# nulltea/hyper-greco

Hardware: AMD Instinct MI355X
Metric: GKR prove ms, n=32768 k=16 Goldilocks; achieved HBM GB/s vs roofline (lower is better)
Workload: dtype u64; 1 GPU; GKR prove (sk_encryption_circuit.rs:444-457) of the BFV sk-enc circuit, n=32768 k=16 Goldilocks/GoldilocksExt2, a new witness every step (4 seeded synthetic witnesses in rotation), node tables resident in HBM; witnesses=4, n=32768, k=16, field=goldilocks, parallelism=dp1: one independent proof per GPU, no data-path collective, proof_bytes=149488

## Files before the change

### hyper-greco_amd/csrc/kernels.hip

```cpp
#include <hip/hip_runtime.h>
#include <cstring>
#include <algorithm>
#include <stdexcept>
#include <string>
#include <type_traits>
#include "kernels.hpp"
#include "gl_wide.hpp"
#include "derive_math.hpp"

namespace hg {
namespace dev {

constexpr int TPB = 256;

template <int CTRL, int ROW_MASK>
__device__ __forceinline__ u64 dpp_u64(u64 v) {
    u32 lo = (u32)__builtin_amdgcn_update_dpp(0, (int)(u32)v, CTRL, ROW_MASK, 0xF, false);
    u32 hi = (u32)__builtin_amdgcn_update_dpp(0, (int)(u32)(v >> 32), CTRL, ROW_MASK, 0xF, false);
    return ((u64)hi << 32) | lo;
}
__device__ __forceinline__ u64 wave_sum_u64(u64 v) {
    v = gl_add(v, dpp_u64<0x111, 0xF>(v));
    v = gl_add(v, dpp_u64<0x112, 0xF>(v));
    v = gl_add(v, dpp_u64<0x114, 0xF>(v));
// ... 408 lines not shown
    if (threadIdx.x == 0) for (int w = 1; w < nw; w++) v = e2_add(v, sm[w]);
    return v;
}

constexpr int SM_SLOTS = 96;
extern __shared__ E2 dyn_lds[];
template <int N>
__device__ __forceinline__ void block_sum_multi(E2 (&v)[N], E2* sm ) {
    const int lane = threadIdx.x & 63, wave = threadIdx.x >> 6, nw = (blockDim.x + 63) >> 6;
#pragma unroll
    for (int k = 0; k < N; k++) v[k] = wave_sum(v[k]);
    __syncthreads();
    if (lane == 0) {
#pragma unroll
        for (int k = 0; k < N; k++) sm[wave * N + k] = v[k];
    }
    __syncthreads();
    if (threadIdx.x == 0)
        for (int w = 1; w < nw; w++) {
#pragma unroll
            for (int k = 0; k < N; k++) v[k] = e2_add(v[k], sm[w * N + k]);
        }
}

__device__ __forceinline__ void part_store(E2* p, E2 v) {
    __hip_atomic_store(&p->c0, v.c0, __ATOMIC_RELAXED, __HIP_MEMORY_SCOPE_AGENT);
    __hip_atomic_store(&p->c1, v.c1, __ATOMIC_RELAXED, __HIP_MEMORY_SCOPE_AGENT);
}
__device__ __forceinline__ E2 part_load(const E2* p) {
    return e2(__hip_atomic_load(&p->c0, __ATOMIC_RELAXED, __HIP_MEMORY_SCOPE_AGENT), __hip_atomic_load(&p->c1, __ATOMIC_RELAXED, __HIP_MEMORY_SCOPE_AGENT));
}
__device__ __forceinline__ unsigned* tickets_of(E2* partials) { return reinterpret_cast<unsigned*>(partials + PARTIALS_E2); }
struct NoPost { __device__ __forceinline__ void operator()(E2*) const {} };
template <typename Post = NoPost>
__device__ __forceinline__ void finish_partials(E2* p, int per, unsigned* ticket, E2* __restrict__ out, E2* sm ,
                                                int nblocks = -1, Post post = Post()) {
    __shared__ unsigned s_last;
    if (nblocks < 0) nblocks = (int)gridDim.x;
    if (threadIdx.x == 0) {
#if !defined(HG_STRICT_TICKETS) && defined(__HIP_DEVICE_COMPILE__) && !defined(__gfx950__) && !defined(__gfx942__)
#error "the vmcnt-ordered ticket below is only valid on gfx942 / gfx950 (stores tracked by vmcnt, sc1 stores written through); build other architectures with -DHG_STRICT_TICKETS"
#endif
#ifdef HG_STRICT_TICKETS
        unsigned t = __hip_atomic_fetch_add(ticket, 1u, __ATOMIC_ACQ_REL, __HIP_MEMORY_SCOPE_AGENT);
#else
        asm volatile("s_waitcnt vmcnt(0)" ::: "memory");
        unsigned t = __hip_atomic_fetch_add(ticket, 1u, __ATOMIC_RELAXED, __HIP_MEMORY_SCOPE_AGENT);
#endif
        s_last = (t == (unsigned)nblocks - 1) ? 1u : 0u;
    }
    __syncthreads();
    if (!s_last) return;
    __builtin_amdgcn_fence(__ATOMIC_ACQUIRE, "agent");
    constexpr int PER_MAX = 6;
    for (int v0 = 0; v0 < per; v0 += PER_MAX) {
        E2 a[PER_MAX];
#pragma unroll
        for (int v = 0; v < PER_MAX; v++) a[v] = e2_zero();
        for (int b = threadIdx.x; b < nblocks; b += blockDim.x) {
            E2 t[PER_MAX];
#pragma unroll
            for (int v = 0; v < PER_MAX; v++) if (v0 + v < per) t[v] = part_load(p + (size_t)b * per + v0 + v);
#pragma unroll
            for (int v = 0; v < PER_MAX; v++) if (v0 + v < per) a[v] = e2_add(a[v], t[v]);
        }
#pragma unroll
        for (int v = 0; v < PER_MAX; v++) if (v0 + v < per) a[v] = block_sum_n(a[v], sm);
        if (threadIdx.x == 0) {
            if constexpr (!std::is_same<Post, NoPost>::value) post(a);
#pragma unroll
            for (int v = 0; v < PER_MAX; v++) if (v0 + v < per) out[v0 + v] = a[v];
        }
    }
    if (threadIdx.x == 0) __hip_atomic_store(ticket, 0u, __ATOMIC_RELAXED, __HIP_MEMORY_SCOPE_AGENT);
}

__device__ __forceinline__ void st_io(const StJob& J, int rd, const void*& in, size_t& in_stride, E2*& out) {
    const size_t h = (size_t)1 << (J.nvars - 1 - rd);
    if (rd == 0) { in = J.in; in_stride = J.in_stride; }
    else { in = J.buf[(rd - 1) & 1]; in_stride = 2 * h; }
    out = rd == J.nvars - 1 ? J.final_out : J.buf[rd & 1];
}

__device__ __forceinline__ int find_item(const StItem* __restrict__ items, int nitems, int blk) {
    const int l = threadIdx.x & 63;
    const int b0 = l < nitems ? items[l].blk0 : 0x7fffffff;
    const unsigned long long m = __ballot(b0 <= blk);
    return __builtin_amdgcn_readfirstlane(__popcll(m) - 1);
}
__device__ __forceinline__ int find_item128(const StItem* __restrict__ items, int nitems, int blk) {
    const int l = threadIdx.x & 63;
    const int b0 = l < nitems ? items[l].blk0 : 0x7fffffff, b1 = l + 64 < nitems ? items[l + 64].blk0 : 0x7fffffff;
    const unsigned long long m0 = __ballot(b0 <= blk), m1 = __ballot(b1 <= blk);
    return __builtin_amdgcn_readfirstlane(__popcll(m0) + __popcll(m1) - 1);
}
template <int KIND, typename T, bool SLOT = false, int MODE = 0>
__global__ __launch_bounds__(256) void k_st_step(const StJob* __restrict__ jobs, const StItem* __restrict__ items, int nitems,
                                                 const E2* __restrict__ chal, E2* __restrict__ partials, E2* __restrict__ res) {
    constexpr int NV = KIND == SC_GRANDPROD ? 3 : 2;
    const int y = find_item(items, nitems, blockIdx.x);
    const StItem& I = items[y];
    const StJob& J = jobs[I.job];
    const int h_log2 = I.h_log2, jb_log2 = I.jb_log2;
    const int rd = J.nvars - 1 - h_log2;
    const size_t half = (size_t)1 << h_log2;
    const int nblocks = I.nblk, bx = (int)blockIdx.x - I.blk0;
    const void* in = I.in; const size_t in_stride = I.in_stride; E2* out = I.out;
    E2* sm = dyn_lds;
    E2* red = dyn_lds + SM_SLOTS;
    E2 acc[NV];
#pragma unroll
    for (int t = 0; t < NV; t++) acc[t] = e2_zero();
    if (rd == 0) sc_round_body<KIND, T, true, SLOT>(reinterpret_cast<const T*>(in), in_stride, out, half, J.ntab, half, chal[J.r_off + rd], J.pw, J.pwr, jb_log2, red, acc, bx, nblocks, J.p0_only != 0, J.next_level,
                                                    SLOT ? &J : nullptr);
    else sc_round_body<KIND, T, false, false, true, MODE>(reinterpret_cast<const T*>(in), in_stride, out, half, J.ntab, half, chal[J.r_off + rd], J.pw, J.pwr, jb_log2, red, acc, bx, nblocks, J.p0_only != 0, nullptr,
                                                          J.mirror ? &J : nullptr);
    if constexpr (MODE == 1) return;
    E2* part = partials + (size_t)y * SC_MAX_BLOCKS * NV;
    block_sum_multi<NV>(acc, sm);
    if (threadIdx.x == 0) {
#pragma unroll
        for (int t = 0; t < NV; t++) {
            if (nblocks == 1) res[J.sums_slot + (size_t)rd * NV + t] = acc[t];
            else part_store(part + (size_t)bx * NV + t, acc[t]);
        }
    }
    if (nblocks > 1) finish_partials(part, NV, tickets_of(partials) + y * 32, res + J.sums_slot + (size_t)rd * NV, sm, nblocks);
}
__device__ __forceinline__ u64 limb_word(const u64* __restrict__ input, const uint8_t* __restrict__ seg_lookup, int seg_shift, size_t rows,
                                         const u64* lookup_mask, size_t j) {
    return j < rows ? input[j] & lookup_mask[seg_lookup[j >> seg_shift]] : 0;
}
__device__ __forceinline__ u32 limb_of(u64 word, int c) { return (u32)(word >> (16 * c)) & 0xFFFF; }
template <typename S>
__device__ __forceinline__ ulonglong2 limb_pair(const S& H, size_t j2, int c) {
    if (j2 >= H.rows) return make_ulonglong2(0, 0);
    const ulonglong2 w = *reinterpret_cast<const ulonglong2*>(H.input + j2);
    const u64 m = H.lookup_mask[H.seg_lookup[j2 >> H.seg_shift]];
    return make_ulonglong2(limb_of(w.x & m, c), limb_of(w.y & m, c));
}
LimbSrc limb_src(const LassoDev& L, const u64* input) {
    LimbSrc S;
    memset(&S, 0, sizeof(S));
    S.input = input; S.seg_lookup = L.seg_lookup; S.seg_shift = L.seg_shift; S.rows = L.rows;
    memcpy(S.lookup_mask, L.lookup_mask, sizeof(S.lookup_mask));
    return S;
}
template <bool MIRROR, bool RECOMP, bool SLOT = false>
#ifndef HG_HASH_SLOT_WAVES
#define HG_HASH_SLOT_WAVES 3
#endif
__global__ __launch_bounds__(256) __attribute__((amdgpu_waves_per_eu(SLOT ? HG_HASH_SLOT_WAVES : 3, SLOT ? HG_HASH_SLOT_WAVES : 3))) void k_gp_first_hash(const StJob* __restrict__ job, const StItem* __restrict__ item,
                                                       const E2* __restrict__ chal, E2* __restrict__ partials, E2* __restrict__ res) {
    const StJob& J = *job;
    const StItem& I = *item;
    const GpHashSrc& H = *J.hash_src;
    const int h_log2 = I.h_log2;
    const size_t half = (size_t)1 << h_log2;
    const size_t hN = half << 1;
    const size_t ntiles = half >> 8;
    const int nblocks = I.nblk, bx = (int)blockIdx.x;
    E2* __restrict__ out = I.out;
    const E2 r = chal[J.r_off];
    const bool p0_only = J.p0_only != 0;
    [[maybe_unused]] constexpr bool mirror = MIRROR;
    const u64 gamma = H.gamma, gamma2 = H.gamma2, tau = H.tau;
    E2 acc[3] = {e2_zero(), e2_zero(), e2_zero()};
    for (size_t tile = bx; tile < ntiles; tile += nblocks) {
        const size_t j = (tile << 8) + threadIdx.x;
        const size_t jo = dpos(j, half);
        GpFirstAcc A = gp_first_acc_zero();
        E2 Sx = e2_zero(), Sy = e2_zero();
        u64 p0 = 0, p2 = 0, p3 = 0;
        int cur_chunk = -1;
        u64 c0 = 0, c1 = 0, c2 = 0, c3 = 0;
        u32 a01 = 0, a23 = 0;
        u32 uses_lo = 0, uses_hi = 0;
        if constexpr (RECOMP) {
            if (2 * j < H.rows) uses_lo = (u32)H.lookup_uses[H.seg_lookup[(2 * j) >> H.seg_shift]];
            if (hN + 2 * j < H.rows) uses_hi = (u32)H.lookup_uses[H.seg_lookup[(hN + 2 * j) >> H.seg_shift]];
        }
        [[maybe_unused]] const int sp = SLOT ? (int)((tile << 9) >> H.seg_shift) : 0;
        for (int m = 0; m < (SLOT ? H.nslots : H.nmem); m++) {
            [[maybe_unused]] int slot_v = m;
            int mi = m;
            if constexpr (SLOT) {
                mi = H.rep[(size_t)m * H.npairs + sp];
                if (mi == 255) {
                    store_e2_nt(out + (size_t)(2 * m) * half + jo, e2_zero());
                    store_e2_nt(out + (size_t)(2 * m + 1) * half + jo, e2_zero());
                    continue;
                }
            }
            const GpHashMem M = H.mems[mi];
            if (M.chunk != cur_chunk) {
                cur_chunk = M.chunk;
                const u64* __restrict__ ts = H.ts[cur_chunk];
                ulonglong2 dl, dh;
                if (H.limb_sh) { dl = limb_pair(H, 2 * j, cur_chunk); dh = limb_pair(H, hN + 2 * j, cur_chunk); }
                else {
                    const u64* __restrict__ dim = H.dim[cur_chunk];
                    dl = *reinterpret_cast<const ulonglong2*>(dim + 2 * j); dh = *reinterpret_cast<const ulonglong2*>(dim + hN + 2 * j);
                }
                const ulonglong2 tl = *reinterpret_cast<const ulonglong2*>(ts + 2 * j), th = *reinterpret_cast<const ulonglong2*>(ts + hN + 2 * j);
                c0 = gl_sub(gl_add(dl.x, gl_mul_small(gamma2, (u32)tl.x)), tau); c1 = gl_sub(gl_add(dl.y, gl_mul_small(gamma2, (u32)tl.y)), tau);
                c2 = gl_sub(gl_add(dh.x, gl_mul_small(gamma2, (u32)th.x)), tau); c3 = gl_sub(gl_add(dh.y, gl_mul_small(gamma2, (u32)th.y)), tau);
                if constexpr (RECOMP) { a01 = (u32)dl.x | ((u32)dl.y << 16); a23 = (u32)dh.x | ((u32)dh.y << 16); }
            }
            u32 e0, e1, e2v, e3;
            if constexpr (RECOMP) {
// ... 708 lines not shown
    const size_t len = (size_t)1 << J.len_log2;
    const size_t idx = (size_t)blockIdx.x * blockDim.x + threadIdx.x;
    if (idx >= ((size_t)J.nrows + J.has_s) << J.len_log2) return;
    const int b = (int)(idx >> J.len_log2);
    const size_t p = idx & (len - 1);
    if (b == J.nrows) { J.out[((size_t)(2 * J.nrows) << J.len_log2) + p] = J.in[((size_t)(2 * J.nslots) << J.len_log2) + p]; return; }
    const size_t t = p < len / 2 ? 2 * p : 2 * (p - len / 2) + 1;
    const int sp = (int)(t >> J.sh);
    const int v = J.slot_of[(size_t)b * J.npairs + sp];
    const E2 l = J.in[((size_t)(2 * v) << J.len_log2) + p], r = J.in[((size_t)(2 * v + 1) << J.len_log2) + p];
    J.out[((size_t)(2 * b) << J.len_log2) + p] = b == 0 ? l : e2_mul(J.ratio[(size_t)b * J.npairs + sp], l);
    J.out[((size_t)(2 * b + 1) << J.len_log2) + p] = r;
}
void gp_slot_regroup_jobs(hipStream_t st, const SlotRegroupJob* jobs, int njobs, size_t max_entries) {
    if (njobs) k_gp_slot_regroup_jobs<<<dim3((unsigned)((max_entries + 255) / 256), (unsigned)njobs), 256, 0, st>>>(jobs);
}
SlotRegroupJob gp_slot_regroup_job(const E2* in, E2* out, const uint8_t* slot_of, const E2* ratio, int nrows, int nslots, int npairs, int len_log2, bool has_s) {
    int np_log2 = 0;
    while ((1 << np_log2) < npairs) np_log2++;
    SlotRegroupJob J;
    J.in = in; J.out = out; J.slot_of = slot_of; J.ratio = ratio; J.nrows = nrows; J.nslots = nslots; J.npairs = npairs; J.len_log2 = len_log2; J.sh = len_log2 - np_log2; J.has_s = has_s ? 1 : 0;
    return J;
}
void gp_slot_regroup(hipStream_t st, const E2* in, E2* out, const uint8_t* slot_of, const E2* ratio, int nrows, int nslots, int npairs, int len_log2, bool has_s) {
    int np_log2 = 0;
    while ((1 << np_log2) < npairs) np_log2++;
    const size_t n = ((size_t)nrows + (has_s ? 1 : 0)) << len_log2;
    k_gp_slot_regroup<<<(unsigned)((n + 255) / 256), 256, 0, st>>>(in, out, slot_of, ratio, nrows, nslots, npairs, len_log2, len_log2 - np_log2, has_s ? 1 : 0);
}
int st_tail_whole_rounds(int ntab, int h0) { return ((size_t)(2 * ntab) << h0) * sizeof(E2) <= ST_TAIL_LDS_BYTES ? 1 : 2; }
size_t st_tail_table_bytes(int ntab, int h0, bool fold_first) {
    const size_t l0 = (size_t)ntab << h0;
    return (fold_first && h0 >= 1 && st_tail_whole_rounds(ntab, h0) == 1 ? 2 * l0 : l0 + (l0 >> 1)) * sizeof(E2);
}
void st_tail(hipStream_t st, int kind, const StJob* jobs, const StItem* items, int nitems, size_t table_bytes, const E2* chal, E2* res, bool fold_first) {
    const size_t lds = (SM_SLOTS + 3 * ST_TAIL_THREADS) * sizeof(E2) + table_bytes;
    static const hipError_t a1 = hipFuncSetAttribute((const void*)k_st_tail<SC_GRANDPROD>, hipFuncAttributeMaxDynamicSharedMemorySize, (int)((SM_SLOTS + 3 * ST_TAIL_THREADS) * sizeof(E2) + ST_TAIL_LDS_BYTES));
    static const hipError_t a2 = hipFuncSetAttribute((const void*)k_st_tail<SC_COLLATION>, hipFuncAttributeMaxDynamicSharedMemorySize, (int)((SM_SLOTS + 3 * ST_TAIL_THREADS) * sizeof(E2) + ST_TAIL_LDS_BYTES));
    static const hipError_t a3 = hipFuncSetAttribute((const void*)k_st_tail<SC_GRANDPROD, true>, hipFuncAttributeMaxDynamicSharedMemorySize, (int)((SM_SLOTS + 3 * ST_TAIL_THREADS) * sizeof(E2) + ST_TAIL_LDS_BYTES));
    (void)a1; (void)a2; (void)a3;
    if (kind == SC_GRANDPROD && fold_first) k_st_tail<SC_GRANDPROD, true><<<nitems, ST_TAIL_THREADS, lds, st>>>(jobs, items, chal, res);
    else if (kind == SC_GRANDPROD) k_st_tail<SC_GRANDPROD><<<nitems, ST_TAIL_THREADS, lds, st>>>(jobs, items, chal, res);
    else k_st_tail<SC_COLLATION><<<nitems, ST_TAIL_THREADS, lds, st>>>(jobs, items, chal, res);
}

int st_plan_blocks(StItem* items, int nitems, bool rounds2) {
    size_t total = 0;
    for (int q = 0; q < nitems; q++) total += (size_t)1 << items[q].h_log2;
    int blk = 0;
    for (int q = 0; q < nitems; q++) {
        StItem& I = items[q];
        int jb = 8;
        if (!rounds2 && I.nrounds != 2) while (jb > 2 && (total << (8 - jb)) < st_min_threads()) jb--;
        if (jb > I.h_log2) jb = I.h_log2;
        const size_t ntiles = ((size_t)1 << I.h_log2) >> jb;
        I.jb_log2 = jb;
        I.blk0 = blk;
        I.nblk = (int)std::min<size_t>(ntiles, (size_t)st_max_blocks());
        blk += I.nblk;
    }
    return blk;
}
void st_step(hipStream_t st, int kind, bool base, const StJob* jobs, const StItem* items, int nitems, int grid, const E2* chal,
             E2* partials, E2* res, bool slot, int mode) {
    const int nv = kind == SC_GRANDPROD ? 3 : 2;
    const size_t lds = sc_lds_bytes(nv, 256);
    if (mode) {
        if (kind != SC_GRANDPROD || base || slot) throw std::runtime_error("st_step: split rounds are grand-product rounds on Ext2 tables");
        if (mode == 1) k_st_step<SC_GRANDPROD, E2, false, 1><<<grid, 256, lds, st>>>(jobs, items, nitems, chal, partials, res);
        else k_st_step<SC_GRANDPROD, E2, false, 2><<<grid, 256, lds, st>>>(jobs, items, nitems, chal, partials, res);
        return;
    }
    if (slot) {
        if (kind != SC_GRANDPROD || !base || nitems != 1) throw std::runtime_error("st_step: a slot-form first round is launched alone");
        k_st_step<SC_GRANDPROD, u64, true><<<grid, 256, lds, st>>>(jobs, items, nitems, chal, partials, res);
    } else if (kind == SC_GRANDPROD) {
        if (base) k_st_step<SC_GRANDPROD, u64><<<grid, 256, lds, st>>>(jobs, items, nitems, chal, partials, res);
        else k_st_step<SC_GRANDPROD, E2><<<grid, 256, lds, st>>>(jobs, items, nitems, chal, partials, res);
    } else {
        if (base) k_st_step<SC_COLLATION, u64><<<grid, 256, lds, st>>>(jobs, items, nitems, chal, partials, res);
        else k_st_step<SC_COLLATION, E2><<<grid, 256, lds, st>>>(jobs, items, nitems, chal, partials, res);
    }
}
void st_step2(hipStream_t st, int kind, const StJob* jobs, const StItem* items, int nitems, int grid, const E2* chal, E2* partials, E2* res) {
    if (kind == SC_GRANDPROD) k_st_step2<false><<<grid, 256, sc_lds_bytes(0, 256), st>>>(jobs, items, nitems, chal, partials, res);
    else k_col_step2<<<grid, 256, sc_lds_bytes(0, 256), st>>>(jobs, items, nitems, chal, partials, res);
}
static_assert(HG_TEST_ST_MAX_BLOCKS <= ST_SUMS_PART_BLOCKS && (size_t)ST_SUMS_MAX_ITEMS * ST_SUMS_PART_BLOCKS * 6 <= PARTIALS_E2 && ST_SUMS_MAX_ITEMS * 16 <= PARTIALS_TICKETS,
              "st_sums: the items of a launch share one partials buffer");
void st_sums(hipStream_t st, const StJob* jobs, const StItem* items, int nitems, int grid, const E2* chal, E2* partials, E2* res) {
    if (nitems > ST_SUMS_MAX_ITEMS) throw std::runtime_error("st_sums: too many items in one launch");
    k_st_step2<true><<<grid, 256, sc_lds_bytes(3, 256), st>>>(jobs, items, nitems, chal, partials, res);
}
__device__ __forceinline__ void ps_io(const PsJob& J, int rd, int rounds, int in_buf, int out_buf, int i, const void*& a, const E2*& b, E2*& oa, E2*& ob) {
    const size_t N = (size_t)1 << J.nvars;
    if (in_buf < 0) { a = J.a[i]; b = J.b[i]; }
    else { size_t len = N >> rd; a = J.bufa[in_buf] + (size_t)i * len; b = J.bufb[in_buf] + (size_t)i * len; }
    if (out_buf < 0) { oa = J.fin_a[i]; ob = J.fin_b[i]; }
    else { size_t len = N >> (rd + rounds); oa = J.bufa[out_buf] + (size_t)i * len; ob = J.bufb[out_buf] + (size_t)i * len; }
}

template <typename TA>
__device__ __forceinline__ void ps_round_body(const PsJob& J, int rd, int in_buf, int out_buf, size_t half, E2 r, int jb_log2, E2& a0, E2& a2,
                                              size_t first_tile, size_t tile_step) {
    using V = Val<TA>;
    const int BD = blockDim.x, tid = threadIdx.x;
    const int G = BD >> jb_log2;
    const int jj = tid & ((1 << jb_log2) - 1), g = tid >> jb_log2;
    const size_t ntiles = half >> jb_log2;
    WE2 w0 = we2_zero(), w2 = we2_zero();
    const FoldR fr = fold_r(r);
    bool touched = false;
    for (size_t tile = first_tile; tile < ntiles; tile += tile_step) {
        const size_t j = (tile << jb_log2) + jj;
        const size_t jo = dpos(j, half);
        for (int i = g; i < J.npairs; i += G) {
            touched = true;
            const void* pa; const E2* pb; E2* oa; E2* ob;
            ps_io(J, rd, 1, in_buf, out_buf, i, pa, pb, oa, ob);
            TA xa, ya;
            E2 xb, yb;
            if (in_buf < 0) {
                load_pair<TA>(reinterpret_cast<const TA*>(pa) + 2 * j, xa, ya);
                load_pair<E2>(pb + 2 * j, xb, yb);
            } else {
                load_xy<TA, false>(reinterpret_cast<const TA*>(pa), j, half, xa, ya);
                load_xy<E2, false>(pb, j, half, xb, yb);
            }
            TA da = V::sub(ya, xa);
            E2 db = e2_sub(yb, xb);
            E2 vb = e2_add(yb, db);
            TA va = V::add(ya, da);
            if constexpr (std::is_same<TA, u64>::value) {
                wmac2(w0.A, xb.c0, xa, w0.C, xb.c1, xa);
                wmac2(w2.A, vb.c0, va, w2.C, vb.c1, va);
                const WAcc f0 = wacc_mul_init(xa, fr.r0, da), f1 = wacc_mul_init(0, fr.r1, da);
                store_e2(oa + jo, e2(wreduce(f0), wreduce(f1)));
            } else {
                we2_mac(w0, xb, xa);
                we2_mac(w2, vb, va);
                store_e2(oa + jo, e2_fold_wide(xa, da, fr));
            }
            store_e2(ob + jo, e2_fold_wide(xb, db, fr));
        }
    }
    if (touched) {
        a0 = e2_add(a0, we2_reduce(w0));
        a2 = e2_add(a2, we2_reduce(w2));
    }
}

__device__ __forceinline__ int find_ps_item(const PsItem* __restrict__ items, int nitems, int blk) {
    const int l = threadIdx.x & 63;
    const int b0 = l < nitems ? items[l].blk0 : 0x7fffffff;
    const unsigned long long m = __ballot(b0 <= blk);
    return __builtin_amdgcn_readfirstlane(__popcll(m) - 1);
}
__global__ __launch_bounds__(256) void k_ps_one(const PsJob* __restrict__ jobs, const PsItem* __restrict__ items, int nitems,
                                                const E2* __restrict__ chal, E2* __restrict__ partials, E2* __restrict__ res) {
    const int y = find_ps_item(items, nitems, blockIdx.x);
    const PsItem& I = items[y];
    const PsJob& J = jobs[I.job];
    const int rd = I.rd;
    const int nblocks = I.nblk, bx = (int)blockIdx.x - I.blk0;
    E2* sm = dyn_lds;
    const size_t half = (size_t)1 << (J.nvars - 1 - rd);
// ... 2033 lines not shown
```

### hyper-greco_amd/csrc/kernels.hpp

```cpp
#pragma once
#include <hip/hip_runtime.h>
#include <algorithm>
#include "gl_field.hpp"

namespace hg {
namespace dev {

constexpr int SC_MAX_BLOCKS = 1024;
constexpr size_t PARTIALS_E2 = (size_t)SC_MAX_BLOCKS * 6 * 64;
constexpr int PARTIALS_TICKETS = 64 * 32;
constexpr size_t PARTIALS_BYTES = PARTIALS_E2 * sizeof(E2) + PARTIALS_TICKETS * sizeof(unsigned);
constexpr int PS_MAX_PAIRS = 32;
constexpr int PW_MAX = 128;
constexpr int PW_ENTRY_MAX = 64;

struct Powers { E2 v[PW_MAX]; };
constexpr int MAX_CLAIMS = 32;
struct ClaimSet {
    int n;
    int unit_alpha;
    size_t alpha_off;
    size_t point_off[MAX_CLAIMS];
};

enum ScKind { SC_COLLATION = 0, SC_GRANDPROD = 1 };

struct GpHashMem {
    const u64* ep;
    int chunk;
    int rd_row, wr_row;
    u32 cutoff;
    int mem;
};
struct GpHashSrc {
    const u64* dim[4];
    const u64* ts[4];
    const GpHashMem* mems;
    int nmem;
    u64 gamma, gamma2, tau;
    int seg_shift;
    size_t rows;
    const uint8_t* seg_lookup;
    u64 lookup_uses[32];
    const u64* input;
    int limb_sh;
    u64 lookup_mask[32];
    const uint8_t* slot_of;
    const uint8_t* rep;
    const E2* slotw;
    int npairs, nslots;
    const u64* emit_rd;
    const u64* emit_wr;
};
void gp_slot_regroup(hipStream_t st, const E2* in, E2* out, const uint8_t* slot_of, const E2* ratio, int nrows, int nslots, int npairs, int len_log2, bool has_s = true);
struct SlotRegroupJob { const E2* in; E2* out; const uint8_t* slot_of; const E2* ratio; int nrows, nslots, npairs, len_log2, sh, has_s; };
SlotRegroupJob gp_slot_regroup_job(const E2* in, E2* out, const uint8_t* slot_of, const E2* ratio, int nrows, int nslots, int npairs, int len_log2, bool has_s);
void gp_slot_regroup_jobs(hipStream_t st, const SlotRegroupJob* jobs, int njobs, size_t max_entries);
struct GpClaimEp {
    E2 mu;
    u64 c;
    int nb;
    int nread;
    int has_next, has_claims;
    size_t evals_slot, next_slot, claims_slot;
    const E2* winv;
    const E2* gnext;
};
struct StJob {
    const void* in;
    size_t in_stride;
    E2* buf[2];
    E2* final_out;
    const GpClaimEp* ep;
    int kind, ntab, nvars, base;
    int p0_only;
    const E2* slotw;
    const u64* emit_mask;
    int slot_ng, slot_shift;
    int mirror;
    E2 mk1, mk2;
    size_t r_off;
    size_t sums_slot;
    const GpHashSrc* hash_src;
    u64* next_level;
    E2 pw[PW_MAX];
    E2 pwr[PW_MAX];
};
struct StItem {
    int job;
    int h_log2;
    int jb_log2;
    int blk0, nblk;
    const void* in;
    size_t in_stride;
    E2* out;
    int rd, nrounds;
    int ntab;
};
int st_plan_blocks(StItem* items, int nitems, bool rounds2);
void st_step(hipStream_t st, int kind, bool base, const StJob* jobs, const StItem* items, int nitems, int grid, const E2* chal,
             E2* partials, E2* res, bool slot = false, int mode = 0);
void st_first_hash(hipStream_t st, const StJob* job, const StItem* item, int grid, bool mirror, bool recomp, const E2* chal, E2* partials, E2* res, bool slot = false);
void st_step2(hipStream_t st, int kind, const StJob* jobs, const StItem* items, int nitems, int grid, const E2* chal, E2* partials, E2* res);
constexpr int ST_SUMS_MAX_ITEMS = 128, ST_SUMS_PART_BLOCKS = 512;
void st_sums(hipStream_t st, const StJob* jobs, const StItem* items, int nitems, int grid, const E2* chal, E2* partials, E2* res);
int st_tail_h(int ntab, int nvars);
int st_tail_whole_rounds(int ntab, int h0);
size_t st_tail_table_bytes(int ntab, int h0, bool fold_first);
void st_tail(hipStream_t st, int kind, const StJob* jobs, const StItem* items, int nitems, size_t table_bytes, const E2* chal, E2* res, bool fold_first = false);
constexpr int ST_SUMS_PAIR_MAX_NB = 24;
constexpr int ST_STEP2_MIN_H = 9;

struct PsJob {
    const void* a[PS_MAX_PAIRS];
    const E2* b[PS_MAX_PAIRS];
    E2* fin_a[PS_MAX_PAIRS];
    E2* fin_b[PS_MAX_PAIRS];
    E2* bufa[2];
    E2* bufb[2];
    int npairs, nvars;
    int tail_rd;
    int tail_buf;
    size_t r_off;
    size_t sums_slot;
    int eq_n, eq_single;
    const E2* eq_scal;
    const E2* eq_lo;
    const E2* eq_suf;
    E2* bufA[2];
    E2* eqA0;
};
struct PsEqPoint {
    size_t point_off;
    int w, nvars;
    unsigned hib;
    int kmin;
    E2* lo;
    E2* suf;
};
inline int ps_eq_kmin(int nvars) { int k = nvars - 13 < 9 ? nvars - 13 : 9; return k < 0 ? 0 : k; }
inline size_t ps_eq_lo_entries(int nvars) { return nvars > 8 ? (size_t)(nvars - 8) * 384 : 0; }
inline size_t ps_eq_suf_entries(int nvars) { return ((size_t)2 << (nvars - ps_eq_kmin(nvars))) - 1; }
constexpr int PS_EQ_MAX_VARS = 26;
void ps_eq_prep(hipStream_t st, const PsEqPoint* pts, int npts, const E2* chal);
void ps_eq_A(hipStream_t st, const PsJob* jobs, const int* ids, int nids, size_t max_quads);
struct PsItem {
    int job, jb_log2, blk0, nblk;
    int rd;
    int in_buf, out_buf;
    int pad;
};
int ps_plan_blocks(PsItem* items, int nitems, const PsJob* host_jobs, bool rounds2);
void ps_round(hipStream_t st, bool rounds2, const PsJob* jobs, const PsItem* items, int nitems, int grid, const E2* chal, E2* partials, E2* res, bool eq = false);
void ps_tail(hipStream_t st, const PsJob* jobs, int njobs, const E2* chal, E2* res);
size_t ps_tail_items_max();

struct ScatterEnt { const E2* src; size_t dst; };
void scatter_e2(hipStream_t st, const ScatterEnt* ents, size_t n, E2* dst_base);
void set_e2(hipStream_t st, E2* dst, E2 v);
void stamp(hipStream_t st, unsigned long long* slot);
struct ClearSet { unsigned* p[4]; size_t n[4]; };
void clear_words(hipStream_t st, const ClearSet& c);

void reduce_partials(hipStream_t st, const E2* partials, int nblocks, int nv, E2* out);

struct EqJob {
    E2* out;
    int n;
    const E2* point_dev;
    ClaimSet cs;
    E2* ab;
    int blk0, rows;
    int pblk0;
};
void eq_jobs(hipStream_t st, const EqJob* jobs, int njobs, int max_n, const E2* chal);
__host__ __device__ inline size_t eq_ab_entries(int n) { return 256 + ((size_t)1 << (n > 8 ? n - 8 : 0)); }
struct EqAbGrid { int prep, fill; };
EqAbGrid eq_ab_plan(EqJob* host_jobs, int njobs);
void eq_jobs_ab(hipStream_t st, const EqJob* jobs, int njobs, EqAbGrid grid, const E2* chal);
void eq_jobs_prep(hipStream_t st, const EqJob* jobs, int njobs, EqAbGrid grid, const E2* chal);
void sum_tables(hipStream_t st, E2* out, const E2* tabs, int ntabs, size_t n);

struct LassoDev {
    int nu, alpha, num_lookups, seg_shift;
    size_t rows;
    const uint8_t* seg_lookup;
    u64 lookup_mask[32];
// ... 112 lines not shown
```

### hyper-greco_amd/csrc/prover_sumcheck.inc

```

    static constexpr size_t TAIL_ITEMS = 4096;

    bool hash_recomp = false;
    std::vector<dev::StJob> st_jobs;
    std::vector<int> st_seq;
    std::vector<SlotPlan> st_slot;
    std::vector<int> st_credit_ntab;
    std::vector<double> st_fused_bytes;
    std::vector<std::function<void()>> st_after_seq;
    double pending_level_design = 0, pending_hash_reads = -1, hash_design_reads = 0;
    std::vector<double> st_level_design, st_hash_reads;
    double pending_fused_bytes = 0;
    double pending_fused_model_extra = 0, hash_model_extra = 0;
    std::vector<double> st_fused_model_extra;
    std::vector<dev::ScatterEnt> scatter;
    struct GpEpReq { int job = -1; dev::GpClaimEp ep; std::vector<E2> winv, gnext; };
    std::vector<GpEpReq> gp_eps;

    ScHandle sc_stride(int kind, const void* in, bool base, size_t in_stride, int ntab, int nvars, const dev::Powers& pw, E2* final_out,
                       bool enqueue = true, bool p0_only = false, int seq = 0, u64* next_level = nullptr, const dev::GpHashSrc* hash_src = nullptr,
                       const MirrorSpec* mirror = nullptr, int model_ntab = 0, const SlotPlan* slots = nullptr) {
        ScHandle h;
        h.nv = kind == dev::SC_GRANDPROD ? 3 : 2;
        h.nvars = nvars;
// ... 99 lines not shown
                    it.job = q; it.h_log2 = next_h[q]; it.in = cur_in[q]; it.in_stride = cur_stride[q]; it.out = J.buf[0];
                    lall.items.push_back(it);
                    cur_in[q] = it.out; cur_stride[q] = (size_t)1 << next_h[q];
                    next_h[q]--;
                }
                if (!lall.items.empty()) plan.push_back(lall);
            }
            static const bool no_split = hg_env_on("HG_NO_SPLIT");
            constexpr int split_h = 14;
            const bool may_split = kind == dev::SC_GRANDPROD && !no_split && st == ctx->stream && fork_recorded && world == 1;
            Launch lsum{kind, false, -1, false, 1, {}};
            lsum.mode = 2;
            for (;;) {
                Launch le{kind, false, -1, false, 1, {}}, l2{kind, false, -1, false, 2, {}};
                bool le_small = may_split;
                for (int q = 0; q < nj; q++) {
                    const dev::StJob& J = st_jobs[q];
                    const int h = next_h[q];
                    if (J.kind != kind || h <= h_small[q]) continue;
                    const bool first = J.nvars - 1 == h;
                    if (first && J.hash_src) throw Error("hash-source job without a sequenced first round");
                    dev::StItem it;
                    memset(&it, 0, sizeof(it));
                    it.job = q; it.h_log2 = h; it.in = cur_in[q]; it.in_stride = cur_stride[q];
                    it.out = first ? J.buf[0] : next_out(q);
                    const bool pair = !first && h - 1 > h_small[q] && h >= std::max(dev::ST_STEP2_MIN_H, fuse_min_h);
                    (pair ? l2 : le).items.push_back(it);
                    if (!pair && (first || h > split_h)) le_small = false;
                    next_h[q] = h - (pair ? 2 : 1);
                    cur_in[q] = it.out; cur_stride[q] = (size_t)1 << (pair ? h - 1 : h);
                }
                if (le.items.empty() && l2.items.empty()) break;
                if (!l2.items.empty()) plan.push_back(l2);
                if (!le.items.empty()) {
                    if (le_small) {
                        le.mode = 1;
                        for (auto& it : le.items) {
                            E2* fresh = ctx->alloc_n<E2>((size_t)st_jobs[it.job].ntab << it.h_log2);
                            it.out = fresh;
                            cur_in[it.job] = fresh;
                            lsum.items.push_back(it);
                        }
                    }
                    plan.push_back(le);
                }
            }
            if (!lsum.items.empty()) {
                if (!hg_env_on("HG_SUMS_SINGLE")) {
                    std::vector<dev::StItem> byjob = lsum.items;
                    std::stable_sort(byjob.begin(), byjob.end(), [](const dev::StItem& a, const dev::StItem& b) { return a.job < b.job; });
                    for (size_t k = 0; k < byjob.size(); k++) {
                        dev::StItem it = byjob[k];
                        if (k + 1 < byjob.size() && byjob[k + 1].job == it.job && byjob[k + 1].h_log2 == it.h_log2 - 1 && it.h_log2 >= dev::ST_STEP2_MIN_H &&
                            st_jobs[it.job].ntab / 2 <= dev::ST_SUMS_PAIR_MAX_NB) { it.nrounds = 2; k++; n_sum_pairs++; }
                        else n_sum_singles++;
                        lsum.run.push_back(it);
                    }
                } else n_sum_singles += (int)lsum.items.size();
                plan.push_back(lsum);
            }
            {
                Launch lc{kind, false, 0, true, 0, {}};
                for (int q = 0; q < nj; q++) {
                    const dev::StJob& J = st_jobs[q];
                    if (J.kind != kind || next_h[q] < 0) continue;
                    const int hs = next_h[q];
                    dev::StItem it;
                    memset(&it, 0, sizeof(it));
                    it.job = q; it.in = cur_in[q]; it.in_stride = cur_stride[q];
                    it.rd = J.nvars - 1 - hs; it.nrounds = hs + 1; it.out = J.final_out;
                    if (st_slot[q].tail_ntab) {
                        const SlotPlan& sp = st_slot[q];
                        if (cur_stride[q] != (size_t)2 << hs) throw Error("slot-form job: unexpected table length at the tail");
                        E2* rg = ctx->alloc_n<E2>((size_t)sp.tail_ntab << (hs + 1));
                        regroups.push_back(Regroup{q, (const E2*)cur_in[q], rg, hs + 1});
                        it.in = rg; it.ntab = sp.tail_ntab;
                    }
                    lc.items.push_back(it);
                    next_h[q] = -1;
                }
                if (!lc.items.empty()) plan.push_back(lc);
            }
        }
        if (hg_debug("plan"))
            for (const Launch& L : plan) {
                if (L.after_seq) { fprintf(stderr, "[hg plan] stride kind=%d after_seq=1\n", L.kind); continue; }
                int lo = INT_MAX, hi = INT_MIN;
                for (const dev::StItem& it : L.items) { const int v = L.tail ? it.nrounds : it.h_log2; lo = std::min(lo, v); hi = std::max(hi, v); }
                fprintf(stderr, "[hg plan] stride kind=%d base=%d nrounds=%d mode=%d tail=%d hash=%d items=%zu %s=%d..%d\n", L.kind, L.base ? 1 : 0, L.nrounds,
                        L.mode, L.tail ? 1 : 0, L.hash ? 1 : 0, L.items.size(), L.tail ? "rounds" : "h", lo, hi);
            }
        if (!gp_eps.empty()) {
            std::vector<E2> wts;
            std::vector<dev::GpClaimEp> eps;
            for (const GpEpReq& e : gp_eps) {
                if (e.job < 0 || e.job >= nj || st_jobs[e.job].kind != dev::SC_GRANDPROD) throw Error("grand product: claim epilogue without its job");
                wts.insert(wts.end(), e.winv.begin(), e.winv.end());
                wts.insert(wts.end(), e.gnext.begin(), e.gnext.end());
            }
            E2* d_wts = ctx->alloc_n<E2>(wts.size());
            dev::GpClaimEp* d_eps = ctx->alloc_n<dev::GpClaimEp>(gp_eps.size());
            size_t o = 0;
            for (size_t i = 0; i < gp_eps.size(); i++) {
                dev::GpClaimEp ep = gp_eps[i].ep;
                ep.winv = d_wts + o; o += gp_eps[i].winv.size();
                ep.gnext = d_wts + o; o += gp_eps[i].gnext.size();
                eps.push_back(ep);
                st_jobs[gp_eps[i].job].ep = d_eps + i;
            }
            upload(d_wts, wts.data(), wts.size() * sizeof(E2), "upload claim weights");
            upload(d_eps, eps.data(), eps.size() * sizeof(dev::GpClaimEp), "upload claim epilogues");
            gp_eps.clear();
        }
        dev::StJob* d_jobs = ctx->alloc_n<dev::StJob>(nj);
        upload(d_jobs, st_jobs.data(), (size_t)nj * sizeof(dev::StJob), "upload jobs");
        std::vector<dev::StItem> flat;
        std::vector<size_t> offs;
        std::vector<std::vector<int>> grids(plan.size());
        for (size_t li = 0; li < plan.size(); li++) {
            Launch& L = plan[li];
            std::vector<dev::StItem>& its = L.run.empty() ? L.items : L.run;
            const size_t batch = L.run.empty() ? MAX_BATCH : (size_t)dev::ST_SUMS_MAX_ITEMS;
            if (!L.tail && !L.after_seq)
                for (size_t o = 0; o < its.size(); o += batch)
                    grids[li].push_back(dev::st_plan_blocks(its.data() + o, (int)std::min<size_t>(batch, its.size() - o), L.nrounds == 2));
            offs.push_back(flat.size());
            flat.insert(flat.end(), its.begin(), its.end());
        }
        dev::StItem* d_items = ctx->alloc_n<dev::StItem>(flat.size());
        upload(d_items, flat.data(), flat.size() * sizeof(dev::StItem), "upload step items");
        auto round_bytes = [&](int q, int rd, bool model) {
            const dev::StJob& J = st_jobs[q];
            size_t half = (size_t)1 << (J.nvars - 1 - rd);
            return (double)(model ? st_credit_ntab[q] : J.ntab) * (2.0 * half * ((J.base && rd == 0) ? 8 : 16) + half * 16.0);
        };
        auto design_bytes = [&](int q, int rd, int nrounds, bool tail) {
            const dev::StJob& J = st_jobs[q];
            const size_t half = (size_t)1 << (J.nvars - 1 - rd);
            double b = (double)J.ntab * 2.0 * half * ((J.base && rd == 0) ? 8 : 16);
            if (rd == 0 && st_hash_reads[q] >= 0) b = st_hash_reads[q];
            if (!tail) b += (double)J.ntab * (double)(half >> (nrounds - 1)) * 16.0;
            if (rd == 0) b += st_level_design[q];
            return b;
        };
        for (size_t li = 0; li < plan.size(); li++) {
            const Launch& L = plan[li];
            if (L.kind == dev::SC_GRANDPROD && st_before_gp) { stamp("collation done"); st_before_gp(); st_before_gp = nullptr; stamp("grand products may start"); }
            if (L.after_seq) {
                for (auto& f : st_after_seq) f();
                st_after_seq.clear();
                if (st_before_gp2) { st_before_gp2(); st_before_gp2 = nullptr; }
                continue;
            }
            const std::vector<dev::StItem>& its = L.run.empty() ? L.items : L.run;
            const size_t batch = L.run.empty() ? MAX_BATCH : (size_t)dev::ST_SUMS_MAX_ITEMS;
            for (size_t o = 0; o < its.size(); o += batch) {
                const int cnt = (int)std::min<size_t>(batch, its.size() - o);
                double bytes = 0, model = 0;
                if (L.hash) {
                    const dev::StItem& it = its[o];
                    bytes = round_bytes(it.job, 0, false) + st_fused_bytes[it.job];
                    model = round_bytes(it.job, 0, true) + st_fused_bytes[it.job] + st_fused_model_extra[it.job];
                    ctx->prof_begin(cls_gp_hash, bytes, model, design_bytes(it.job, 0, 1, false));
                    dev::st_first_hash(st, d_jobs + it.job, d_items + offs[li] + o, grids[li][0], st_jobs[it.job].mirror != 0, hash_recomp, ctx->d_chal, partials, d_res(), st_slot[it.job].tail_ntab != 0);
                    ctx->prof_end();
                    stamp("first hash round done");
                    continue;
                }
                if (L.tail) {
                    size_t table_bytes = 0;
                    double design = 0;
                    const bool tail_ff = L.kind == dev::SC_GRANDPROD && !hg_env_on("HG_TAIL_WHOLE_ROUNDS");
                    std::vector<dev::SlotRegroupJob> rg_jobs;
                    size_t rg_max = 0;
                    for (int q = 0; q < cnt; q++) {
                        const dev::StItem& it = its[o + q];
                        const dev::StJob& J = st_jobs[it.job];
                        for (int k = 0; k < it.nrounds; k++) { bytes += round_bytes(it.job, it.rd + k, false); model += round_bytes(it.job, it.rd + k, true); }
                        design += (double)(it.ntab > 0 ? it.ntab : J.ntab) * 2.0 * (double)((size_t)1 << (J.nvars - 1 - it.rd)) * ((J.base && it.rd == 0) ? 8 : 16);
                        const int h0 = J.nvars - 1 - it.rd, tn = it.ntab > 0 ? it.ntab : J.ntab;
                        table_bytes = std::max(table_bytes, dev::st_tail_table_bytes(tn, h0, tail_ff));
                        if (tail_ff && it.nrounds > dev::st_tail_whole_rounds(tn, h0)) n_tail_ff++;
                        else if (L.kind == dev::SC_GRANDPROD) n_tail_whole++;
                        for (const Regroup& g : regroups) if (g.job == it.job) {
                            const SlotPlan& sp = st_slot[it.job];
                            rg_jobs.push_back(dev::gp_slot_regroup_job(g.in, g.out, sp.d_slot_of, sp.d_ratio, sp.nrows, sp.nslots, sp.npairs, g.len_log2, (sp.tail_ntab & 1) != 0));
                            rg_max = std::max(rg_max, ((size_t)sp.nrows + (sp.tail_ntab & 1)) << g.len_log2);
                        }
                    }
                    if (!rg_jobs.empty()) {
                        dev::SlotRegroupJob* d_rg = ctx->alloc_n<dev::SlotRegroupJob>(rg_jobs.size());
                        upload(d_rg, rg_jobs.data(), rg_jobs.size() * sizeof(dev::SlotRegroupJob), "upload regroup jobs");
                        dev::gp_slot_regroup_jobs(st, d_rg, (int)rg_jobs.size(), rg_max);
                    }
                    ctx->prof_begin(cls_tail, bytes, model, design);
                    dev::st_tail(st, L.kind, d_jobs, d_items + offs[li] + o, cnt, table_bytes, ctx->d_chal, d_res(), tail_ff);
                    ctx->prof_end();
                } else {
                    double design = 0;
                    for (int q = 0; q < cnt; q++) {
                        const dev::StItem& it = its[o + q];
                        const dev::StJob& J = st_jobs[it.job];
                        design += design_bytes(it.job, J.nvars - 1 - it.h_log2, L.nrounds, false);
                        for (int k = 0; k < L.nrounds; k++) { bytes += round_bytes(it.job, J.nvars - 1 - it.h_log2 + k, false); model += round_bytes(it.job, J.nvars - 1 - it.h_log2 + k, true); }
                        if (L.base && it.h_log2 == J.nvars - 1) { bytes += st_fused_bytes[it.job]; model += st_fused_bytes[it.job]; }
                    }
                    const int grid = grids[li][o / batch];
                    int cls = L.kind == dev::SC_GRANDPROD ? (L.base ? cls_gp_base : (L.nrounds == 2 ? cls_gp_ext2 : cls_gp_ext)) : (L.base ? cls_col_base : (L.nrounds == 2 ? cls_col_ext2 : cls_col_ext));
                    if (L.mode == 2) {
                        if (o == 0) {
                            hip_check(hipEventRecord(ctx->ev_sum[0], st), "split rounds: folds done");
                            hip_check(hipStreamWaitEvent(ctx->stream_sum, ctx->ev_sum[0], 0), "split rounds: wait for the folds");
                        }
                        ctx->prof_stream = ctx->stream_sum;
                        ctx->prof_begin(cls_gp_sums, 0, 0, design);
                        if (!L.run.empty()) dev::st_sums(ctx->stream_sum, d_jobs, d_items + offs[li] + o, cnt, grid, ctx->d_chal, ctx->d_partials4, d_res());
                        else dev::st_step(ctx->stream_sum, L.kind, false, d_jobs, d_items + offs[li] + o, cnt, grid, ctx->d_chal, ctx->d_partials4, d_res(), false, 2);
                        ctx->prof_end();
                        ctx->prof_stream = st;
                        if (o + batch >= its.size()) {
                            hip_check(hipEventRecord(ctx->ev_sum[1], ctx->stream_sum), "split rounds: sums done");
                            ctx->sum_pending = true;
                        }
                        continue;
                    }
                    ctx->prof_begin(cls, bytes, model, design);
                    if (L.nrounds == 2) dev::st_step2(st, L.kind, d_jobs, d_items + offs[li] + o, cnt, grid, ctx->d_chal, partials, d_res());
                    else dev::st_step(st, L.kind, L.base, d_jobs, d_items + offs[li] + o, cnt, grid, ctx->d_chal, partials, d_res(),
                                      L.base && st_jobs[its[o].job].slotw != nullptr, L.mode);
                    ctx->prof_end();
                }
            }
        }
        if (hg_debug("endgame") && (n_tail_ff || n_tail_whole || n_sum_pairs || n_sum_singles))
            fprintf(stderr, "[hg endgame] stride tail_fold_first=%d tail_whole=%d sums_pairs=%d sums_singles=%d\n", n_tail_ff, n_tail_whole, n_sum_pairs, n_sum_singles);
        if (st_before_gp) { st_before_gp(); st_before_gp = nullptr; }
        if (st_before_gp2) { st_before_gp2(); st_before_gp2 = nullptr; }
        st_jobs.clear();
        st_seq.clear();
        st_credit_ntab.clear();
        st_slot.clear();
        st_fused_bytes.clear();
        st_fused_model_extra.clear();
        st_level_design.clear();
        st_hash_reads.clear();
        for (auto& f : st_after_seq) f();
        st_after_seq.clear();
        if (!scatter.empty()) {
            dev::ScatterEnt* d = ctx->alloc_n<dev::ScatterEnt>(scatter.size());
            upload(d, scatter.data(), scatter.size() * sizeof(dev::ScatterEnt), "upload scatter list");
            dev::scatter_e2(st, d, scatter.size(), d_res());
            scatter.clear();
        }
    }

    std::map<int, std::vector<dev::PsJob>> ps_queue;
    std::vector<std::function<void()>> second_wave;

    ScHandle sc_prodsum(const std::vector<const u64*>& a, const std::vector<const E2*>& b, int nvars,
                        const std::vector<E2*>& fin_a, const std::vector<E2*>& fin_b, bool enqueue = true) {
        ScHandle h;
        h.nv = 2;
        h.nvars = nvars;
        h.point_off = epos();
        h.sums_slot = slot((size_t)nvars * 2);
        if (!enqueue) {
            for (int i = 0; i < nvars; i++) h.rs.push_back(squeeze());
            return h;
        }
        const int np = (int)a.size();
        if (np > dev::PS_MAX_PAIRS) throw Error("prodsum: too many table pairs");
        const size_t N = (size_t)1 << nvars;
        dev::PsJob J;
        memset(&J, 0, sizeof(J));
        J.npairs = np; J.nvars = nvars; J.r_off = h.point_off; J.sums_slot = h.sums_slot;
        for (int q = 0; q < 2; q++) {
            J.bufa[q] = ctx->alloc_n<E2>((size_t)np * std::max<size_t>(N >> (q + 1), 1));
            J.bufb[q] = ctx->alloc_n<E2>((size_t)np * std::max<size_t>(N >> (q + 1), 1));
        }
        for (int i = 0; i < np; i++) { J.a[i] = a[i]; J.b[i] = b[i]; J.fin_a[i] = fin_a[i]; J.fin_b[i] = fin_b[i]; }
        for (int i = 0; i < nvars; i++) h.rs.push_back(squeeze());
        ps_queue[nvars].push_back(J);
        return h;
    }
    static bool ps_eq_on() { static const bool v = !hg_env_on("HG_NO_PS_EQ"); return v; }
    static size_t ps_tail_items() { return std::min<size_t>(TAIL_ITEMS, dev::ps_tail_items_max()); }
    static int eq_tail_rd(int npairs, int nvars) {
        if (npairs < 1 || npairs > dev::PS_MAX_PAIRS || nvars > dev::PS_EQ_MAX_VARS) return -1;
        const size_t N = (size_t)1 << nvars;
        int rd = 0;
        while (rd < nvars && ((N >> rd) / 2) * (size_t)npairs > ps_tail_items()) rd++;
        if (rd & 1) rd++;
        if (rd < 2 || rd > nvars - 8 || rd < dev::ps_eq_kmin(nvars)) return -1;
        return rd;
    }
    std::vector<E2> eq_scal_host;
    std::vector<dev::PsEqPoint> eqpt_queue;
    std::map<std::tuple<size_t, int, int, unsigned>, std::pair<E2*, E2*>> eqpt_shared;
    ScHandle sc_prodsum_eq(const std::vector<const u64*>& a, const std::vector<E2>& kappa, const std::vector<E2>& zp, size_t z_off, int w, unsigned hib,
                           int nvars, int tail_rd, const std::vector<E2*>& fin_a, const std::vector<E2*>& fin_b, bool enqueue) {
        ScHandle h;
        h.nv = 2;
        h.nvars = nvars;
        h.point_off = epos();
        h.sums_slot = slot((size_t)nvars * 2);
        for (int i = 0; i < nvars; i++) h.rs.push_back(squeeze());
        if (!enqueue) return h;
        const int np = (int)a.size();
        const size_t N = (size_t)1 << nvars;
        dev::PsJob J;
        memset(&J, 0, sizeof(J));
        J.npairs = np; J.nvars = nvars; J.r_off = h.point_off; J.sums_slot = h.sums_slot;
        J.tail_rd = tail_rd; J.eq_n = np; J.eq_single = np == 1 ? 1 : 0;
        for (int q = 0; q < 2; q++) {
            J.bufa[q] = ctx->alloc_n<E2>((size_t)np * (N >> (q + 1)));
            if (np > 1) J.bufA[q] = ctx->alloc_n<E2>(N >> (q + 1));
        }
        if (np > 1) J.eqA0 = ctx->alloc_n<E2>(N);
// ... 465 lines not shown
```

Before: 1.473 ms.

## Fuse consecutive fold-only sumcheck rounds into one tiled LDS kernel

Adds a kernel that takes a run of consecutive fold-only (mode 1) grand-product rounds per job and performs up to ten folds per 512-entry tile in LDS. It reads the input table once and writes each round's output from shared memory, with a software-prefetched next tile. Previously each of these rounds was a separate launch that re-read the prior round's output from HBM. The goal is fewer launches and less HBM re-read traffic, at the cost of syncthreads-heavy tail levels where most threads sit idle. It is on by default and can be disabled with HG_FOLD_ROUNDS.

Result: faster. 1.397 ms, median of 6 (-5.2%).

```diff
diff --git a/hyper-greco_amd/csrc/kernels.hip b/hyper-greco_amd/csrc/kernels.hip
--- a/hyper-greco_amd/csrc/kernels.hip
+++ b/hyper-greco_amd/csrc/kernels.hip
@@ -514,7 +514,8 @@
     out = rd == J.nvars - 1 ? J.final_out : J.buf[rd & 1];
 }
 
-__device__ __forceinline__ int find_item(const StItem* __restrict__ items, int nitems, int blk) {
+template <typename Item>
+__device__ __forceinline__ int find_item(const Item* __restrict__ items, int nitems, int blk) {
     const int l = threadIdx.x & 63;
     const int b0 = l < nitems ? items[l].blk0 : 0x7fffffff;
     const unsigned long long m = __ballot(b0 <= blk);
@@ -558,6 +559,62 @@
         }
     }
     if (nblocks > 1) finish_partials(part, NV, tickets_of(partials) + y * 32, res + J.sums_slot + (size_t)rd * NV, sm, nblocks);
+}
+__global__ __launch_bounds__(256) void k_st_fold_runs(const StJob* __restrict__ jobs, const StFoldRun* __restrict__ items, int nitems, const E2* __restrict__ chal) {
+    constexpr int NL = (1 << ST_FOLD_TILE_MAX_LOG2) / 256 > 0 ? (1 << ST_FOLD_TILE_MAX_LOG2) / 256 : 1;
+    static_assert((1 << ST_FOLD_TILE_MAX_LOG2) <= 2 * 256, "k_st_fold_runs: level 1 of a tile is one entry per thread");
+    __shared__ E2 lv0[1 << ST_FOLD_TILE_MAX_LOG2], lv1[1 << (ST_FOLD_TILE_MAX_LOG2 - 1)];
+    const int y = find_item(items, nitems, blockIdx.x);
+    const StFoldRun& I = items[y];
+    const StJob& J = jobs[I.job];
+    const int h0 = I.h0, nr = I.nrounds, p = I.tile_log2, P = 1 << p, tid = threadIdx.x;
+    const int nblk = I.nblk, bx = (int)blockIdx.x - I.blk0;
+    const size_t half0 = (size_t)1 << h0, units = (size_t)J.ntab << (h0 - p);
+    const E2* rch = chal + J.r_off + (J.nvars - 1 - h0);
+    const E2* in = I.in; const size_t in_stride = I.in_stride;
+    auto fetch = [&](size_t u, E2* x, E2* yv) {
+        const size_t tab = u >> (h0 - p), j0 = (u & ((half0 >> p) - 1)) << p;
+#pragma unroll
+        for (int q = 0; q < NL; q++) if (tid + q * 256 < P) load_xy<E2, false>(in + tab * in_stride, j0 + tid + q * 256, half0, x[q], yv[q]);
+    };
+    E2 cx[NL], cy[NL];
+    if ((size_t)bx < units) fetch(bx, cx, cy);
+    for (size_t u = bx; u < units; u += nblk) {
+        const size_t tab = u >> (h0 - p), j0 = (u & ((half0 >> p) - 1)) << p;
+        E2 nx[NL], ny[NL];
+        if (u + nblk < units) fetch(u + nblk, nx, ny);
+        {
+            const FoldR fr = fold_r(rch[0]);
+#pragma unroll
+            for (int q = 0; q < NL; q++) {
+                const int l = tid + q * 256;
+                if (l < P) {
+                    const E2 v = e2_fold_wide(cx[q], e2_sub(cy[q], cx[q]), fr);
+                    if (nr == 1) store_e2(I.out[0] + tab * half0 + dpos(j0 + l, half0), v);
+                    else lv0[l] = v;
+                }
+            }
+        }
+        for (int k = 1; k < nr; k++) {
+            __syncthreads();
+            const E2* src = (k & 1) ? lv0 : lv1;
+            E2* dst = (k & 1) ? lv1 : lv0;
+            const size_t hk = half0 >> k;
+            if (tid < (P >> k)) {
+                const size_t jk = (j0 >> k) + tid;
+                const E2 x = src[2 * tid], yv = src[2 * tid + 1];
+                E2* lo = I.out[k - 1] + tab * (2 * hk);
+                store_e2(lo + jk, x);
+                store_e2(lo + hk + jk, yv);
+                const E2 v = e2_fold_wide(x, e2_sub(yv, x), fold_r(rch[k]));
+                if (k == nr - 1) store_e2(I.out[k] + tab * hk + dpos(jk, hk), v);
+                else dst[tid] = v;
+            }
+        }
+        __syncthreads();
+#pragma unroll
+        for (int q = 0; q < NL; q++) { cx[q] = nx[q]; cy[q] = ny[q]; }
+    }
 }
 __device__ __forceinline__ u64 limb_word(const u64* __restrict__ input, const uint8_t* __restrict__ seg_lookup, int seg_shift, size_t rows,
                                          const u64* lookup_mask, size_t j) {
@@ -1432,6 +1489,23 @@
         else k_st_step<SC_COLLATION, E2><<<grid, 256, lds, st>>>(jobs, items, nitems, chal, partials, res);
     }
 }
+int st_plan_fold_blocks(StFoldRun* items, int nitems, const StJob* host_jobs, int tile_log2) {
+    if (nitems > 64 || tile_log2 < 1 || tile_log2 > ST_FOLD_TILE_MAX_LOG2) throw std::runtime_error("st_plan_fold_blocks: items or tile out of range");
+    int blk = 0;
+    for (int q = 0; q < nitems; q++) {
+        StFoldRun& I = items[q];
+        I.tile_log2 = std::min(tile_log2, I.h0);
+        if (I.h0 < 0 || I.nrounds < 1 || I.nrounds > I.tile_log2 + 1) throw std::runtime_error("st_plan_fold_blocks: a run longer than its tile holds");
+        const size_t units = (size_t)host_jobs[I.job].ntab << (I.h0 - I.tile_log2);
+        I.blk0 = blk;
+        I.nblk = (int)std::min<size_t>(units, (size_t)st_max_blocks());
+        blk += I.nblk;
+    }
+    return blk;
+}
+void st_fold_runs(hipStream_t st, const StJob* jobs, const StFoldRun* items, int nitems, int grid, const E2* chal) {
+    k_st_fold_runs<<<grid, 256, 0, st>>>(jobs, items, nitems, chal);
+}
 void st_step2(hipStream_t st, int kind, const StJob* jobs, const StItem* items, int nitems, int grid, const E2* chal, E2* partials, E2* res) {
     if (kind == SC_GRANDPROD) k_st_step2<false><<<grid, 256, sc_lds_bytes(0, 256), st>>>(jobs, items, nitems, chal, partials, res);
     else k_col_step2<<<grid, 256, sc_lds_bytes(0, 256), st>>>(jobs, items, nitems, chal, partials, res);
diff --git a/hyper-greco_amd/csrc/kernels.hpp b/hyper-greco_amd/csrc/kernels.hpp
--- a/hyper-greco_amd/csrc/kernels.hpp
+++ b/hyper-greco_amd/csrc/kernels.hpp
@@ -103,6 +103,19 @@
 void st_first_hash(hipStream_t st, const StJob* job, const StItem* item, int grid, bool mirror, bool recomp, const E2* chal, E2* partials, E2* res, bool slot = false);
 void st_step2(hipStream_t st, int kind, const StJob* jobs, const StItem* items, int nitems, int grid, const E2* chal, E2* partials, E2* res);
 constexpr int ST_SUMS_MAX_ITEMS = 128, ST_SUMS_PART_BLOCKS = 512;
+constexpr int ST_FOLD_TILE_MAX_LOG2 = 9, ST_FOLD_MAX_ROUNDS = ST_FOLD_TILE_MAX_LOG2 + 1;
+constexpr int ST_FOLD_TILE_LOG2 = 9;
+struct StFoldRun {
+    int job;
+    int h0, nrounds;
+    int tile_log2;
+    int blk0, nblk;
+    const E2* in;
+    size_t in_stride;
+    E2* out[ST_FOLD_MAX_ROUNDS];
+};
+int st_plan_fold_blocks(StFoldRun* items, int nitems, const StJob* host_jobs, int tile_log2);
+void st_fold_runs(hipStream_t st, const StJob* jobs, const StFoldRun* items, int nitems, int grid, const E2* chal);
 void st_sums(hipStream_t st, const StJob* jobs, const StItem* items, int nitems, int grid, const E2* chal, E2* partials, E2* res);
 int st_tail_h(int ntab, int nvars);
 int st_tail_whole_rounds(int ntab, int h0);
diff --git a/hyper-greco_amd/csrc/prover_sumcheck.inc b/hyper-greco_amd/csrc/prover_sumcheck.inc
--- a/hyper-greco_amd/csrc/prover_sumcheck.inc
+++ b/hyper-greco_amd/csrc/prover_sumcheck.inc
@@ -205,6 +205,43 @@
                 if (!lc.items.empty()) plan.push_back(lc);
             }
         }
+        int fold_at = -1, fold_tile = dev::ST_FOLD_TILE_LOG2, fold_rounds = 0, fold_max_run = 0;
+        struct FoldLaunch { size_t off; int cnt, grid; double bytes, model, design; };
+        std::vector<FoldLaunch> fold_launches;
+        std::vector<dev::StFoldRun> fold_items;
+        if (!hg_env_on("HG_FOLD_ROUNDS")) {
+            if (const char* e = getenv("HG_FOLD_TILE_LOG2")) { const int v = atoi(e); if (v >= 1 && v <= dev::ST_FOLD_TILE_MAX_LOG2) fold_tile = v; }
+            std::vector<std::vector<dev::StItem>> runs(nj);
+            for (size_t li = 0; li < plan.size(); li++)
+                if (plan[li].mode == 1) { fold_at = (int)li; for (const dev::StItem& it : plan[li].items) runs[it.job].push_back(it); }
+            std::vector<std::vector<dev::StFoldRun>> pieces;
+            for (int q = 0; q < nj; q++) {
+                const std::vector<dev::StItem>& run = runs[q];
+                for (size_t k = 1; k < run.size(); k++)
+                    if (run[k].h_log2 != run[k - 1].h_log2 - 1 || run[k].in != (const void*)run[k - 1].out || run[k].in_stride != (size_t)1 << run[k - 1].h_log2)
+                        throw Error("fold-only rounds of a job that do not follow each other");
+                fold_rounds += (int)run.size();
+                fold_max_run = std::max(fold_max_run, (int)run.size());
+                size_t c = 0;
+                for (size_t pos = 0; pos < run.size(); c++) {
+                    dev::StFoldRun F;
+                    memset(&F, 0, sizeof(F));
+                    F.job = q; F.h0 = run[pos].h_log2; F.in = (const E2*)run[pos].in; F.in_stride = run[pos].in_stride;
+                    F.nrounds = (int)std::min<size_t>((size_t)std::min(fold_tile, F.h0) + 1, run.size() - pos);
+                    for (int k = 0; k < F.nrounds; k++) F.out[k] = run[pos + k].out;
+                    if (pieces.size() <= c) pieces.emplace_back();
+                    pieces[c].push_back(F);
+                    pos += (size_t)F.nrounds;
+                }
+            }
+            for (const auto& pc : pieces)
+                for (size_t o = 0; o < pc.size(); o += MAX_BATCH) {
+                    FoldLaunch FL{fold_items.size(), (int)std::min<size_t>(MAX_BATCH, pc.size() - o), 0, 0, 0, 0};
+                    fold_items.insert(fold_items.end(), pc.begin() + o, pc.begin() + o + FL.cnt);
+                    FL.grid = dev::st_plan_fold_blocks(fold_items.data() + FL.off, FL.cnt, st_jobs.data(), fold_tile);
+                    fold_launches.push_back(FL);
+                }
+        }
         if (hg_debug("plan"))
             for (const Launch& L : plan) {
                 if (L.after_seq) { fprintf(stderr, "[hg plan] stride kind=%d after_seq=1\n", L.kind); continue; }
@@ -266,9 +303,33 @@
             if (rd == 0) b += st_level_design[q];
             return b;
         };
+        dev::StFoldRun* d_fold = nullptr;
+        if (!fold_items.empty()) {
+            d_fold = ctx->alloc_n<dev::StFoldRun>(fold_items.size());
+            upload(d_fold, fold_items.data(), fold_items.size() * sizeof(dev::StFoldRun), "upload fold runs");
+            for (FoldLaunch& FL : fold_launches)
+                for (int q = 0; q < FL.cnt; q++) {
+                    const dev::StFoldRun& F = fold_items[FL.off + q];
+                    const dev::StJob& J = st_jobs[F.job];
+                    FL.design += (double)J.ntab * 2.0 * (double)((size_t)1 << F.h0) * 16.0;
+                    for (int k = 0; k < F.nrounds; k++) {
+                        FL.bytes += round_bytes(F.job, J.nvars - 1 - F.h0 + k, false); FL.model += round_bytes(F.job, J.nvars - 1 - F.h0 + k, true);
+                        FL.design += (double)J.ntab * (double)((size_t)1 << (F.h0 - k)) * 16.0;
+                    }
+                }
+        }
         for (size_t li = 0; li < plan.size(); li++) {
             const Launch& L = plan[li];
             if (L.kind == dev::SC_GRANDPROD && st_before_gp) { stamp("collation done"); st_before_gp(); st_before_gp = nullptr; stamp("grand products may start"); }
+            if (L.mode == 1 && fold_at >= 0) {
+                if ((int)li == fold_at)
+                    for (const FoldLaunch& FL : fold_launches) {
+                        ctx->prof_begin(cls_gp_ext, FL.bytes, FL.model, FL.design);
+                        dev::st_fold_runs(st, d_jobs, d_fold + FL.off, FL.cnt, FL.grid, ctx->d_chal);
+                        ctx->prof_end();
+                    }
+                continue;
+            }
             if (L.after_seq) {
                 for (auto& f : st_after_seq) f();
                 st_after_seq.clear();
@@ -357,6 +418,8 @@
         }
         if (hg_debug("endgame") && (n_tail_ff || n_tail_whole || n_sum_pairs || n_sum_singles))
             fprintf(stderr, "[hg endgame] stride tail_fold_first=%d tail_whole=%d sums_pairs=%d sums_singles=%d\n", n_tail_ff, n_tail_whole, n_sum_pairs, n_sum_singles);
+        if (hg_debug("folds") && !fold_launches.empty())
+            fprintf(stderr, "[hg folds] stride launches=%zu items=%zu rounds=%d max_run=%d tile_log2=%d\n", fold_launches.size(), fold_items.size(), fold_rounds, fold_max_run, fold_tile);
         if (st_before_gp) { st_before_gp(); st_before_gp = nullptr; }
         if (st_before_gp2) { st_before_gp2(); st_before_gp2 = nullptr; }
         st_jobs.clear();
```
